# ORNL-Fusion/graph_framework

Measured on AMD Instinct MI355X. Metric: ray-steps/sec on xrays_bench cold-plasma; achieved HBM GB/s vs peak, higher is better.
Workload: dtype f64

## Files before the change

graph_framework_amd/build.py:

```python
import glob
import os
import subprocess

from . import _lib

HIPCC = os.environ.get("HIPCC", "/opt/rocm/bin/hipcc")
KERNEL_FLAGS = ["-O3", "-ffp-contract=off", "-fno-slp-vectorize", "--offload-arch=gfx950"]


def build_library(force=False):
    csrc = os.path.join(_lib.HERE, "csrc")
    sources = glob.glob(os.path.join(csrc, "*")) + glob.glob(os.path.join(_lib.HERE, "..", "include", "*.h"))
    newest = max(os.path.getmtime(s) for s in sources)
    programs = [os.path.join(_lib.HERE, name) for name in ("xrays_bench", "solver_check", "korc_push")]
    sources.append(os.path.join(_lib.HERE, "gf_workflow.hpp"))
    newest = max(os.path.getmtime(s) for s in sources)
    if (force or not os.path.exists(_lib.LIB_PATH) or os.path.getmtime(_lib.LIB_PATH) < newest
            or any(not os.path.exists(p) or os.path.getmtime(p) < newest for p in programs)):
        subprocess.check_call(["make", "-C", csrc, "-s", "HIPCC=" + HIPCC])
    return _lib.LIB_PATH


def compile_source(source, source_hash, force=False):
    os.makedirs(_lib.CACHE_DIR, exist_ok=True)
    stem = os.path.join(_lib.CACHE_DIR, "%016x" % source_hash)
    if force or not os.path.exists(stem + ".hsaco"):
        with open(stem + ".hip", "w") as f:
            f.write(source)
        subprocess.check_call([HIPCC, "--genco"] + KERNEL_FLAGS + ["-o", stem + ".hsaco", stem + ".hip"])
    return stem + ".hsaco"


def prebuild_kernel(gfir_path, force=False):
    from . import backend
    return [compile_source(source, source_hash, force) for source, source_hash in backend.generate_piece_sources(gfir_path)]


VARIANTS = [({"GFHIP_DIVISION": "fast"}, "solver_kernel_f64"), ({"GFHIP_DIVISION": "fast"}, "loss_kernel_kx_f64"),
            ({"GFHIP_ASM": "0"}, "solver_kernel_f64")]


def variant_sources():
    import json
    import sys
    texts = []
    for overrides, stem in VARIANTS:
        env = dict(os.environ)
        env.update(overrides)
        out = subprocess.run([sys.executable, "-c",
                              "import sys, json; sys.path.insert(0, %r)\n"
                              "from graph_framework_amd.backend import generate_piece_sources\n"
                              "print(json.dumps(generate_piece_sources(%r)))"
                              % (os.path.dirname(_lib.HERE), os.path.join(_lib.WORKLOAD_DIR, stem + ".gfir"))],
                             env=env, capture_output=True, text=True, check=True)
        texts += [tuple(piece) for piece in json.loads(out.stdout)]
    return texts


def prebuild_workloads(force=False):
    from concurrent.futures import ThreadPoolExecutor
    from . import backend
    paths = sorted(glob.glob(os.path.join(_lib.WORKLOAD_DIR, "*.gfir")))
# ... 15 lines not shown
```

graph_framework_amd/csrc/asm_body.hpp:

```cpp
#ifndef gfhip_asm_body_hpp
#define gfhip_asm_body_hpp

#include <algorithm>
#include <cstdint>
#include <cstdio>
#include <cstring>
#include <map>
#include <set>
#include <sstream>
#include <string>
#include <tuple>
#include <vector>

#include "gfir_item.hpp"
#include "options.hpp"
#include "schedule.hpp"
#include "tables.hpp"

namespace gfhip {

struct asm_body_text {
    bool ok = false;
    std::string why;
    std::string statement;
    uint32_t slots = 0;
    size_t vector = 0, scalar = 0, lds_reads = 0, lds_writes = 0, loads = 0, waits = 0;
};

class asm_body_writer {
    const item &it;
    const codegen_options &opt;
    const std::vector<pack> &packs;
    const std::vector<int> &parent;
    const std::vector<double> &factor;
    const std::vector<uint32_t> &table_pack, &table_column;
    const uint32_t block_size;
    const uint32_t slot_limit;
// ... 150 lines not shown
        used_at.assign(n, std::vector<int64_t> ());
        node_group.assign(n, -1);
        for (size_t i = 0; i < n; i++) {
            const gfir_instruction &c = it.code[i];
            alias[i] = static_cast<int64_t> (i);
            if (c.op == GFIR_GATHER1 || c.op == GFIR_GATHER2) {
                const table &t = it.tables[c.aux];
                const bool two = c.op == GFIR_GATHER2;
                const group_key key(c.a, two ? c.b : GFIR_NONE, t.rows, t.cols, c.imm[0], c.imm[1], two ? c.imm[2] : 0.0, two ? c.imm[3] : 0.0);
                auto found = group_of_key.find(key);
                if (found == group_of_key.end()) {
                    group g;
                    g.pack = table_pack[c.aux];
                    groups.push_back(g);
                    found = group_of_key.insert({key, static_cast<int> (groups.size()) - 1}).first;
                }
                node_group[i] = found->second;
                alias[i] = cell_value(found->second, c.aux);
            }
        }
        std::vector<bool> group_seen(groups.size(), false);
        for (size_t i = 0; i < n; i++) {
            const gfir_instruction &c = it.code[i];
            if (c.op == GFIR_CONST || c.op == GFIR_INPUT) continue;
            if (c.op == GFIR_GATHER1 || c.op == GFIR_GATHER2) {
                const size_t g = static_cast<size_t> (node_group[i]);
                if (!group_seen[g]) {
                    group_seen[g] = true;
                    if (it.code[c.a].op != GFIR_CONST) add_use(alias[c.a], i);
                    if (c.op == GFIR_GATHER2 && it.code[c.b].op != GFIR_CONST) add_use(alias[c.b], i);
                }
                continue;
            }
            const uint32_t operands[3] = {c.a, c.b, c.c};
            for (int k = 0; k < operand_count(c.op); k++) {
                if (it.code[operands[k]].op != GFIR_CONST) add_use(alias[operands[k]], i);
            }
            if (c.op == GFIR_DIV) add_use(static_cast<int64_t> (n + c.b), i);
        }
        for (auto &st : it.setters) {
            if (it.code[st.value].op != GFIR_CONST) add_use(alias[st.value], n);
        }
        for (auto o : it.outputs) {
            if (it.code[o].op != GFIR_CONST) add_use(alias[o], n);
        }
        for (size_t k = 2*n; k < values.size(); k++) {
            int64_t child = static_cast<int64_t> (k);
// ... 452 lines not shown
                vector_op("v_mad_u32_u24 " + low_name(cell) + ", " + low_name(index[0]) + ", " + std::to_string(t.cols) + ", " + low_name(index[1]));
            } else {
                vector_op("v_mul_u32_u24_e32 " + low_name(cell) + ", " + hex32(t.cols) + ", " + low_name(index[0]));
                vector_op("v_add_u32_e32 " + low_name(cell) + ", " + low_name(cell) + ", " + low_name(index[1]));
            }
            release_pair(index[1]);
        }
        const std::string defines = "def g" + std::to_string(node_group[i]) + " node " + std::to_string(i) + " stride " + std::to_string(pk.stride*8u) +
                                    " pack " + std::to_string(g.pack) + " lds " + std::to_string(pk.in_lds ? 1 : 0);
        if (!pk.in_lds) annotate(defines);
        vector_op("v_mul_u32_u24_e32 " + low_name(cell) + ", " + hex32(pk.stride*8u) + ", " + low_name(cell));
        if (pk.in_lds) {
            annotate(defines);
            vector_op("v_add_u32_e32 " + low_name(cell) + ", %[lds" + std::to_string(g.pack) + "], " + low_name(cell));
        }
        g.offset_pair = cell;
        owner[static_cast<size_t> (cell)] = -2;
    }

    void node(const size_t i) {
        const gfir_instruction &c = it.code[i];
        position = i;
        pinned.clear();
        look_ahead();
        std::vector<int64_t> read = used_at[i];
        switch (c.op) {
            case GFIR_CONST:
                return;
            case GFIR_INPUT:
                values[i].operand = "%[v" + std::to_string(c.a) + "]";
                values[i].defined = true;
                return;
            case GFIR_GATHER1:
            case GFIR_GATHER2:
                if (groups[static_cast<size_t> (node_group[i])].offset_pair == -1) find_cell(i);
                line("; alias r" + std::to_string(i) + " = " + value_name(alias[i]));
                break;
            case GFIR_ADD:
            case GFIR_SUB:
            case GFIR_MUL:
            case GFIR_FMA: {
                operands x = c.op == GFIR_FMA ? resolve({c.a, c.b, c.c}) : resolve({c.a, c.b}, {false, c.op == GFIR_SUB});
                retire(read);
                read.clear();
                const int p = need_pair();
                const char *name = c.op == GFIR_MUL ? "v_mul_f64 " : c.op == GFIR_FMA ? "v_fma_f64 " : "v_add_f64 ";
// ... 201 lines not shown
                if (k) s << ", ";
                s << "[park" << k << "] \"v\"(park" << k << ")";
            }
        }
        s << "\n                : ";
        for (uint32_t r = pool_lo; r < 256; r++) s << "\"v" << r << "\", ";
        for (int r = sgpr_lo; r < sgpr_lo + 2*sgpr_pairs; r++) s << "\"s" << r << "\", ";
        s << "\"memory\");\n";
        result.statement = s.str();
        result.ok = true;
        return result;
    }
};

inline item schedule_for_assembly(const item &in, const codegen_options &opt, const std::vector<std::string> &directories = {}) {
    if (in.code.size() > 20000 || !asm_body_writer::why_not(in, opt).empty()) return schedule_for_pressure(in);
    if (const char *forced = std::getenv("GFHIP_ASM_SEED")) {
        return reorder(in, list_schedule(in, static_cast<uint32_t> (std::atoi(forced))));
    }
    const std::vector<uint8_t> bytes = in.serialize();
    const uint64_t key = fnv1a(std::string(bytes.begin(), bytes.end()) + "|order|" + std::to_string(opt.asm_pool_lo) + "|" +
                               std::to_string(opt.asm_load_ahead) + "|" + std::to_string(opt.asm_reload_ahead) + "|" +
                               std::to_string(opt.asm_schedule_tries) + "|" + std::to_string(opt.asm_wide_loads) + "|" +
                               std::to_string(opt.lds_budget) + "|" + std::to_string(opt.compact_tables) + "|" + std::to_string(opt.block_size));
    char name[40];
    std::snprintf(name, sizeof(name), "/%016llx.order", static_cast<unsigned long long> (key));
    for (auto &directory : directories) {
        if (FILE *f = std::fopen((directory + name).c_str(), "r")) {
            unsigned int seed = 0;
            const bool read = std::fscanf(f, "%u", &seed) == 1;
            std::fclose(f);
            if (read) return reorder(in, list_schedule(in, seed));
        }
    }
    const table_layout layout = layout_tables(in, opt);
    item best;
    uint32_t best_seed = 0;
    size_t best_slots = ~static_cast<size_t> (0), best_traffic = 0;
    const uint32_t tries = in.code.size() <= 5000 ? opt.asm_schedule_tries
                         : std::max<uint32_t> (4u, static_cast<uint32_t> (opt.asm_schedule_tries*5000ull/in.code.size()));
    for (uint32_t seed = 0; seed < std::max(1u, tries); seed++) {
        item candidate = reorder(in, list_schedule(in, seed));
        asm_body_writer writer(candidate, opt, layout.packs, layout.parent, layout.factor, layout.table_pack, layout.table_column,
                               opt.block_size, 1u << 20);
        const asm_body_text text = writer.write();
        if (!text.ok) continue;
        const size_t traffic = text.lds_reads + text.lds_writes;
        if (std::getenv("GFHIP_ASM_REPORT")) {
            std::fprintf(stderr, "  order %u of %s: %u slots, %zu LDS reads, %zu LDS writes, %zu loads, %zu waits\n", seed, in.name.c_str(), text.slots,
                         text.lds_reads, text.lds_writes, text.loads, text.waits);
        }
        if (text.slots < best_slots || (text.slots == best_slots && traffic < best_traffic)) {
            best_slots = text.slots;
            best_traffic = traffic;
            best = std::move(candidate);
            best_seed = seed;
        }
    }
    if (best.code.empty()) return schedule_for_pressure(in);
    for (auto &directory : directories) {
        if (FILE *f = std::fopen((directory + name).c_str(), "w")) {
            std::fprintf(f, "%u\n", best_seed);
            std::fclose(f);
            break;
        }
    }
// ... 16 lines not shown
```

graph_framework_amd/csrc/codegen.hpp:

```cpp
#ifndef gfhip_codegen_hpp
#define gfhip_codegen_hpp

#include <algorithm>
#include <cmath>
#include <cstdint>
#include <cstdio>
#include <cstdlib>
#include <functional>
#include <map>
#include <set>
#include <sstream>
#include <string>
#include <tuple>
#include <vector>

#include "asm_body.hpp"
#include "gfir_item.hpp"
#include "options.hpp"
#include "parking.hpp"
#include "prelude.hpp"
#include "schedule.hpp"
#include "tables.hpp"

namespace gfhip {
// ... 129 lines not shown
            [&] (const std::string &group, const uint32_t t) -> std::string {
            const std::string value_name = "c" + group.substr(1) + "_" + std::to_string(t);
            if (coefficients.insert(value_name).second) {
                if (parent[t] >= 0) {
                    const std::string from = value_at(group, static_cast<uint32_t> (parent[t]));
                    s << ind << "const real " << value_name << " = " << literal(factor[t]) << "*" << from << ";\n";
                } else {
                    s << ind << "const real " << value_name << " = " << group << "[" << table_column[t] << "u];\n";
                }
            }
            return value_name;
        };
        std::map<uint32_t, std::pair<std::string, uint32_t>> deferred;
        auto define = [&] (const uint32_t v) {
            auto found = deferred.find(v);
            if (found == deferred.end()) return;
            const std::string value = value_at(found->second.first, found->second.second);
            s << ind << "const real r" << v << " = " << value << ";\n";
            deferred.erase(found);
        };
        for (size_t i = 0; i < it.code.size(); i++) {
            const gfir_instruction &c = it.code[i];
            reload(i);
            {
                const uint32_t operands[3] = {c.a, c.b, c.c};
                for (int k = 0; k < operand_count(c.op); k++) define(operands[k]);
            }
            switch (c.op) {
                case GFIR_CONST:
                    s << ind << "const real r" << i << " = " << value_literal(c.imm[0], c.imm[1]) << ";\n";
                    break;
                case GFIR_RANDOM:
                    s << ind << "const real r" << i << " = gf_from_base(static_cast<base> (gf_random(random_state)));\n";
                    break;
                case GFIR_INPUT:
                    s << ind << "const real r" << i << " = v" << c.a << ";\n";
                    break;
                case GFIR_ADD:
                    s << ind << "const real r" << i << " = " << N(c.a) << " + " << N(c.b) << ";\n";
                    break;
                case GFIR_SUB:
                    s << ind << "const real r" << i << " = " << N(c.a) << " - " << N(c.b) << ";\n";
                    break;
                case GFIR_MUL:
                    s << ind << "const real r" << i << " = ";
                    if (safe) s << "(" << N(c.a) << " == " << value_literal(0.0) << " || " << N(c.b) << " == " << value_literal(0.0) << ") ? " << value_literal(0.0) << " : ";
// ... 498 lines not shown
          << "        const real other = __shfl_down(" << lane << ", offset, 64);\n"
          << "        " << lane << " = other > " << lane << " ? other : " << lane << ";\n"
          << "    }\n"
          << "    __shared__ real " << scratch << "[" << out.block_size/64 << "];\n"
          << "    if ((threadIdx.x & 63u) == 0u) " << scratch << "[threadIdx.x >> 6] = " << lane << ";\n"
          << "    __syncthreads();\n"
          << "    if (threadIdx.x == 0u) {\n"
          << "        real block_max = " << scratch << "[0];\n"
          << "        for (unsigned int w = 1; w < (blockDim.x >> 6); w++) block_max = " << scratch << "[w] > block_max ? " << scratch << "[w] : block_max;\n"
          << "        const " << bits << " b = __builtin_bit_cast(" << bits << ", block_max);\n"
          << "        const " << bits << " top = static_cast<" << bits << "> (1) << " << (f64 ? 63 : 31) << ";\n"
          << "        atomicMax(" << target << ", static_cast<unsigned long long> (block_max != block_max ? static_cast<" << bits << "> (~static_cast<" << bits << "> (0))\n"
          << "                                                             : (b & top) ? static_cast<" << bits << "> (~b) : (b | top)));\n"
          << "    }\n";
    }
};

inline lowered lower(const item &original, const codegen_options &opt = codegen_options::from_environment(),
                     const piece_info &piece = piece_info()) {
    item scheduled;
    if (opt.schedule_for_pressure && !(opt.asm_body && piece.scheduled)) {
        scheduled = schedule_for_pressure(original);
    }
    const item &it = scheduled.code.empty() ? original : scheduled;
    lowered out;
    const size_t esize = it.element_size();

    out.input_written.assign(it.symbols.size(), false);
    for (auto &s : it.setters) {
        out.input_written[s.input] = true;
    }

    const table_layout layout = layout_tables(it, opt);
    const std::vector<int> &parent = layout.parent;
    const std::vector<double> &factor = layout.factor;
    const std::vector<uint32_t> &table_pack = layout.table_pack, &table_column = layout.table_column;
    out.table_parent = parent;
    out.table_factor = factor;
    out.packs = layout.packs;
    size_t lds_used = layout.lds_used;
    out.block_size = opt.block_size;

    const bool generic = it.is_complex() || it.safe_math() || it.has_random();
    codegen_options plain = opt;
    if (generic) plain.park_in_lds = false;
    asm_body_text assembly;
// ... 77 lines not shown
```

graph_framework_amd/csrc/gf_hip.cpp:

```cpp
#include <hip/hip_runtime.h>
#include <hip/hiprtc.h>

#include <dlfcn.h>
#include <sys/stat.h>

#include <cmath>
#include <complex>
#include <cstdio>
#include <cstdlib>
#include <cstring>
#include <fstream>
#include <limits>
#include <map>
#include <memory>
#include <optional>
#include <string>
#include <type_traits>
#include <vector>

#include "../../include/gf_hip.h"
#include "codegen.hpp"
#include "segments.hpp"

#include "converge_state.hpp"
#include "superacc.hpp"

namespace gfhip {
void launch_max_reduce(const void *in, const size_t n, const bool f64,
                       unsigned long long *result, const unsigned int num_cus, hipStream_t stream);
void launch_converge_decide(const bool f64, unsigned long long *reduced, void *state, hipStream_t stream);
void launch_converge_decide_batch(const bool f64, unsigned long long *reduced, void *state, const unsigned int count, hipStream_t stream);
void launch_max_modulus(const void *in, const size_t n, const bool f64, void *result, hipStream_t stream);
void launch_deposit(const double *x, const double *y, const double *z, const double *value, const size_t count,
                    const double *edges, const int nx, const int ny, const int nz, const double *scale,
                    void *state, unsigned long long *counters, const unsigned int num_cus, hipStream_t stream);
void launch_bins_normalise(void *state, const size_t cells, hipStream_t stream);
void launch_bins_round(const void *state, const size_t cells, const double divisor, double *bins, hipStream_t stream);
void launch_bins_merge(void *state, const void *other, const size_t words, hipStream_t stream);
}

namespace {

thread_local std::string creation_error;

// ... 234 lines not shown

static uint32_t plan_item(const gfhip::item &it, gfhip::lowered &whole, std::vector<built_piece> &pieces,
                          std::optional<built_piece> *redo = nullptr) {
    const gfhip::codegen_options opt = gfhip::codegen_options::from_environment();
    size_t count = 1;
    bool automatic = false;
    if (gfhip::can_split(it)) {
        if (opt.segments >= 1 && it.code.size() >= opt.segments_min_nodes && it.code.size() >= 2*opt.segments) {
            count = opt.segments;
        } else if (opt.segment_nodes && it.code.size() > opt.segment_nodes) {
            count = (it.code.size() + opt.segment_nodes - 1)/opt.segment_nodes;
            automatic = true;
        }
    }
    bool as_assembly = opt.asm_body && count < 2 && opt.segments == 0 && opt.schedule_for_pressure && gfhip::can_split(it) &&
                       it.code.size() >= opt.asm_min_nodes && opt.division == gfhip::division_mode::shared &&
                       gfhip::asm_body_writer::why_not(it, opt).empty();
    gfhip::item ordered;
    if (as_assembly) {
        std::vector<std::string> directories;
        if (const char *env = std::getenv("GFHIP_CACHE_DIR")) directories.push_back(env);
        directories.push_back(library_directory() + "/kernel_cache");
        ordered = gfhip::schedule_for_assembly(it, opt, directories);
        as_assembly = gfhip::assembly_fits(ordered, opt);
    }
    if (count < 2 && opt.segments != 1 && !as_assembly) {
        whole = gfhip::lower(it, opt);
        return 0;
    }
    if (!as_assembly) ordered = opt.schedule_for_pressure ? gfhip::schedule_for_pressure(it) : it;
    gfhip::segmentation plan = gfhip::split_item(ordered, gfhip::choose_cuts(ordered, count));
    if (plan.segments.size() == 1) plan.segments[0].piece.name = it.name;
    gfhip::codegen_options piece_options = opt;
    if (automatic) piece_options.division = gfhip::division_mode::ieee;
    const bool with_redo = !automatic && piece_options.division != gfhip::division_mode::ieee;
    std::vector<bool> after_division(ordered.code.size(), false);
    for (size_t i = 0; i < ordered.code.size(); i++) {
        const gfir_instruction &c = ordered.code[i];
        const uint32_t operands[3] = {c.a, c.b, c.c};
        bool dependent = c.op == GFIR_DIV;
        for (int k = 0; k < gfhip::operand_count(c.op) && !dependent; k++) dependent = after_division[operands[k]];
        after_division[i] = dependent;
    }
    for (size_t p = 0; p < plan.segments.size(); p++) {
        built_piece piece;
        gfhip::piece_info role;
        role.scheduled = opt.schedule_for_pressure;
        if (with_redo) {
            role.role = p + 1 == plan.segments.size() ? gfhip::piece_role::last : gfhip::piece_role::middle;
            for (auto slot : plan.segments[p].output_slot) role.output_handed_over.push_back(slot >= 0);
            for (auto record : plan.segments[p].symbol_record) role.symbol_after_division.push_back(record >= 0 && after_division[record]);
        }
        piece.low = gfhip::lower(plan.segments[p].piece, piece_options, role);
// ... 1228 lines not shown
```

graph_framework_amd/csrc/gfir_item.hpp:

```cpp
#ifndef gfir_item_hpp
#define gfir_item_hpp

#include <cctype>
#include <cstdint>
#include <cstring>
#include <string>
#include <vector>

#include "../../include/gfir.h"

namespace gfhip {

struct table {
    uint32_t rows, cols;
    std::vector<double> data;
};

struct item {
    uint32_t dtype = GFIR_F64;
    uint32_t flags = 0;
    std::string name;
    std::vector<std::string> symbols;
    std::vector<table> tables;
    std::vector<gfir_instruction> code;
    std::vector<uint32_t> outputs;
    std::vector<gfir_setter> setters;

    static size_t element_size(const uint32_t dtype) {
        return dtype == GFIR_F32 ? 4 : dtype == GFIR_C64 ? 16 : 8;
    }
    size_t element_size() const { return element_size(dtype); }
    bool is_complex() const { return dtype == GFIR_C32 || dtype == GFIR_C64; }
    bool base_is_f64() const { return dtype == GFIR_F64 || dtype == GFIR_C64; }
    bool safe_math() const { return flags & GFIR_SAFE_MATH; }
    bool has_random() const {
        for (auto &c : code) {
            if (c.op == GFIR_RANDOM) return true;
        }
        return false;
    }

    size_t indexed_length(const uint32_t i) const {
        size_t length = 0;
        for (auto &c : code) {
            if ((c.op == GFIR_INDEX1 || c.op == GFIR_INDEX2) && c.c == i) {
                const size_t needed = c.op == GFIR_INDEX1 ? c.aux : static_cast<size_t> (c.aux)*c.reserved;
                if (needed > length) length = needed;
            }
        }
// ... 187 lines not shown
```

graph_framework_amd/csrc/options.hpp:

```cpp
#ifndef gfhip_options_hpp
#define gfhip_options_hpp

#include <cstdint>
#include <cstdlib>
#include <string>

namespace gfhip {

enum class division_mode {
    shared,
    checked,
    ieee,
    fast
};

struct codegen_options {
    size_t lds_budget = 64*1024;
    uint32_t block_size = 256;
    uint32_t waves_per_simd = 0;
    division_mode division = division_mode::shared;
    bool pow_three_halves = true;
    bool window_sqrt = false;
    bool window_sqrt_f32 = true;
    int nontemporal = -1;
    bool compact_tables = true;
    bool park_in_lds = true;
    uint32_t park_min_range = 1500;
    uint32_t park_window = 100;
    uint32_t park_max_slots = 32;
    uint32_t park_prefetch = 50;
    uint32_t park_capacity = 0;
    bool schedule_for_pressure = true;
    int division_fixup = -1;
    uint32_t converge_batch = 3;
    uint32_t segment_nodes = 6000;
    uint32_t segments = 0;
    uint32_t segments_min_nodes = 2000;
    bool asm_body = true;
    uint32_t asm_waves = 2;
    bool asm_wide_loads = true;
    uint32_t asm_schedule_tries = 64;
    uint32_t asm_min_nodes = 1000;
    uint32_t asm_pool_lo = 40;
    uint32_t asm_load_ahead = 96;
    uint32_t asm_reload_ahead = 24;
    size_t handover_bytes = 128u << 20;

    static codegen_options from_environment() {
        codegen_options o;
        if (const char *e = std::getenv("GFHIP_DIVISION")) {
            const std::string mode(e);
            o.division = mode == "ieee" ? division_mode::ieee : mode == "checked" ? division_mode::checked
                       : mode == "fast" ? division_mode::fast : division_mode::shared;
        }
        if (const char *e = std::getenv("GFHIP_PARK")) {
            const std::string mode(e);
            o.park_in_lds = mode != "0";
            if (mode == "heavy") o.park_min_range = 300;
        }
        if (const char *e = std::getenv("GFHIP_SCHEDULE")) o.schedule_for_pressure = std::string(e) != "source";
        if (const char *e = std::getenv("GFHIP_DIV_FIXUP")) o.division_fixup = std::string(e) != "0" ? 1 : 0;
        if (const char *e = std::getenv("GFHIP_NONTEMPORAL")) o.nontemporal = std::atoi(e);
        if (const char *e = std::getenv("GFHIP_COMPACT_TABLES")) o.compact_tables = std::string(e) != "0";
        if (const char *e = std::getenv("GFHIP_POW")) o.pow_three_halves = std::string(e) != "libm";
        if (const char *e = std::getenv("GFHIP_PARK_CAPACITY")) o.park_capacity = static_cast<uint32_t> (std::atoi(e));
        if (const char *e = std::getenv("GFHIP_PARK_PREFETCH")) o.park_prefetch = static_cast<uint32_t> (std::atoi(e));
        if (const char *e = std::getenv("GFHIP_ASM")) o.asm_body = std::string(e) != "0";
        if (const char *e = std::getenv("GFHIP_ASM_WAVES")) o.asm_waves = static_cast<uint32_t> (std::atoi(e)) == 2 ? 2 : 1;
        if (const char *e = std::getenv("GFHIP_ASM_WIDE_LOADS")) o.asm_wide_loads = std::string(e) != "0";
        if (const char *e = std::getenv("GFHIP_ASM_TRIES")) o.asm_schedule_tries = static_cast<uint32_t> (std::atoi(e));
        if (const char *e = std::getenv("GFHIP_ASM_MIN_NODES")) o.asm_min_nodes = static_cast<uint32_t> (std::atoi(e));
        if (const char *e = std::getenv("GFHIP_ASM_POOL_LO")) o.asm_pool_lo = static_cast<uint32_t> (std::atoi(e));
        if (const char *e = std::getenv("GFHIP_ASM_LOAD_AHEAD")) o.asm_load_ahead = static_cast<uint32_t> (std::atoi(e));
        if (const char *e = std::getenv("GFHIP_ASM_RELOAD_AHEAD")) o.asm_reload_ahead = static_cast<uint32_t> (std::atoi(e));
        if (const char *e = std::getenv("GFHIP_WINDOW_SQRT")) o.window_sqrt = std::string(e) == "1";
        if (const char *e = std::getenv("GFHIP_WINDOW_SQRT_F32")) o.window_sqrt_f32 = std::string(e) == "1";
        if (const char *e = std::getenv("GFHIP_WAVES_PER_SIMD")) o.waves_per_simd = static_cast<uint32_t> (std::atoi(e));
        if (const char *e = std::getenv("GFHIP_LDS_BUDGET")) o.lds_budget = static_cast<size_t> (std::atol(e));
        if (const char *e = std::getenv("GFHIP_CONVERGE_BATCH")) o.converge_batch = static_cast<uint32_t> (std::atol(e) > 0 ? std::atol(e) : 1);
        if (o.converge_batch > 8) o.converge_batch = 8;
        if (const char *e = std::getenv("GFHIP_SEGMENT_NODES")) o.segment_nodes = static_cast<uint32_t> (std::atol(e));
        if (const char *e = std::getenv("GFHIP_SEGMENTS")) o.segments = static_cast<uint32_t> (std::atol(e));
        if (const char *e = std::getenv("GFHIP_SEGMENTS_MIN_NODES")) o.segments_min_nodes = static_cast<uint32_t> (std::atol(e));
        if (const char *e = std::getenv("GFHIP_HANDOVER_BYTES")) o.handover_bytes = static_cast<size_t> (std::atoll(e));
        return o;
    }
};

inline uint64_t fnv1a(const std::string &s) {
    uint64_t h = 1469598103934665603ull;
    for (unsigned char c : s) {
        h ^= c;
        h *= 1099511628211ull;
    }
    return h;
}

inline const char *compile_flags() {
    return "-O3 -ffp-contract=off -fno-slp-vectorize --offload-arch=gfx950";
}

}

#endif
```

graph_framework_amd/csrc/schedule.hpp:

```cpp
#ifndef gfhip_schedule_hpp
#define gfhip_schedule_hpp

#include <set>
#include <vector>

#include "gfir_item.hpp"

namespace gfhip {

inline int operand_count(const uint32_t op) {
    switch (op) {
        case GFIR_CONST: case GFIR_INPUT: return 0;
        case GFIR_FMA: return 3;
        case GFIR_SQRT: case GFIR_POWI: case GFIR_SIN: case GFIR_COS: case GFIR_EXP: case GFIR_LOG: case GFIR_ERFI:
        case GFIR_GATHER1: case GFIR_INDEX1: case GFIR_RANDOM: return 1;
        default: return 2;
    }
}

inline item reorder(const item &in, const std::vector<uint32_t> &order) {
    const size_t n = in.code.size();
    std::vector<uint32_t> new_index(n, GFIR_NONE);
    for (size_t p = 0; p < order.size(); p++) new_index[order[p]] = static_cast<uint32_t> (p);
    item out = in;
    for (size_t p = 0; p < order.size(); p++) {
        gfir_instruction c = in.code[order[p]];
        const int count = operand_count(c.op);
        if (count > 0) c.a = new_index[c.a];
        if (count > 1) c.b = new_index[c.b];
        if (count > 2) c.c = new_index[c.c];
        out.code[p] = c;
    }
    for (auto &s : out.setters) s.value = new_index[s.value];
    for (auto &o : out.outputs) o = new_index[o];
    return out;
}

inline item schedule_for_pressure(const item &in) {
    const size_t n = in.code.size();
    if (n > 20000) return in;
    std::vector<std::vector<uint32_t>> users(n);
    std::vector<uint32_t> pending(n, 0), consumers_left(n, 0);
    std::vector<bool> is_root(n, false);
    for (auto &s : in.setters) is_root[s.value] = true;
    for (auto o : in.outputs) is_root[o] = true;
    for (size_t i = 0; i < n; i++) {
        const gfir_instruction &c = in.code[i];
        const uint32_t operands[3] = {c.a, c.b, c.c};
        std::set<uint32_t> distinct;
        for (int k = 0; k < operand_count(c.op); k++) distinct.insert(operands[k]);
        pending[i] = static_cast<uint32_t> (distinct.size());
        for (auto o : distinct) {
            users[o].push_back(static_cast<uint32_t> (i));
            consumers_left[o]++;
        }
    }

    std::vector<uint32_t> distinct_operands(3*n, GFIR_NONE);
    std::vector<uint8_t> distinct_count(n, 0);
    for (size_t i = 0; i < n; i++) {
        const gfir_instruction &c = in.code[i];
        const uint32_t operands[3] = {c.a, c.b, c.c};
        for (int k = 0; k < operand_count(c.op); k++) {
            bool seen = false;
            for (int j = 0; j < distinct_count[i]; j++) seen = seen || distinct_operands[3*i + j] == operands[k];
            if (!seen) distinct_operands[3*i + distinct_count[i]++] = operands[k];
        }
    }

    std::set<uint32_t> ready;
    std::vector<uint32_t> stamp(n, 0);
    for (size_t i = 0; i < n; i++) {
        if (pending[i] == 0) ready.insert(static_cast<uint32_t> (i));
    }
    std::vector<uint32_t> order;
    order.reserve(n);
    while (!ready.empty()) {
        uint32_t best = *ready.begin();
        int best_score = 1 << 30;
        for (const uint32_t v : ready) {
            int freed = 0;
            for (int k = 0; k < distinct_count[v]; k++) {
                const uint32_t o = distinct_operands[3*static_cast<size_t> (v) + k];
                if (in.code[o].op != GFIR_CONST && consumers_left[o] == 1 && !is_root[o]) freed++;
            }
            const int grows = (in.code[v].op == GFIR_CONST) ? 0 : 1;
            const int score = grows - freed;
            if (score < best_score || (score == best_score && stamp[v] > stamp[best])) {
                best_score = score;
                best = v;
            }
        }
        ready.erase(best);
        order.push_back(best);
        for (int k = 0; k < distinct_count[best]; k++) consumers_left[distinct_operands[3*static_cast<size_t> (best) + k]]--;
        for (auto u : users[best]) {
            if (--pending[u] == 0) {
                ready.insert(u);
                stamp[u] = static_cast<uint32_t> (order.size());
            }
        }
    }

    return reorder(in, order);
}

inline std::vector<uint32_t> list_schedule(const item &in, const uint32_t seed) {
    const size_t n = in.code.size();
    uint64_t state = 0x9E3779B97F4A7C15ull*(seed + 1u);
    auto next = [&state] () {
        uint64_t z = (state += 0x9E3779B97F4A7C15ull);
        z = (z ^ (z >> 30))*0xBF58476D1CE4E5B9ull;
        z = (z ^ (z >> 27))*0x94D049BB133111EBull;
        return z ^ (z >> 31);
    };
    std::vector<std::vector<uint32_t>> users(n);
    std::vector<uint32_t> pending(n, 0), consumers_left(n, 0);
    std::vector<bool> is_root(n, false);
    for (auto &s : in.setters) is_root[s.value] = true;
    for (auto o : in.outputs) is_root[o] = true;
    std::vector<uint32_t> distinct_operands(3*n, GFIR_NONE);
    std::vector<uint8_t> distinct_count(n, 0);
    for (size_t i = 0; i < n; i++) {
        const gfir_instruction &c = in.code[i];
        const uint32_t operands[3] = {c.a, c.b, c.c};
        for (int k = 0; k < operand_count(c.op); k++) {
            bool seen = false;
            for (int j = 0; j < distinct_count[i]; j++) seen = seen || distinct_operands[3*i + j] == operands[k];
            if (!seen) distinct_operands[3*i + distinct_count[i]++] = operands[k];
        }
        pending[i] = distinct_count[i];
        for (int k = 0; k < distinct_count[i]; k++) {
            users[distinct_operands[3*i + k]].push_back(static_cast<uint32_t> (i));
            consumers_left[distinct_operands[3*i + k]]++;
        }
    }
    std::set<uint32_t> ready;
    std::vector<uint32_t> stamp(n, 0), order, best;
    for (size_t i = 0; i < n; i++) {
        if (pending[i] == 0) ready.insert(static_cast<uint32_t> (i));
    }
    order.reserve(n);
    while (!ready.empty()) {
        best.clear();
        int best_score = 1 << 30;
        uint32_t best_stamp = 0;
        for (const uint32_t v : ready) {
            int freed = 0;
            for (int k = 0; k < distinct_count[v]; k++) {
                const uint32_t o = distinct_operands[3*static_cast<size_t> (v) + k];
                if (in.code[o].op != GFIR_CONST && consumers_left[o] == 1 && !is_root[o]) freed++;
            }
            const int score = (in.code[v].op == GFIR_CONST ? 0 : 1) - freed;
            if (score < best_score || (score == best_score && stamp[v] > best_stamp)) {
                best_score = score;
                best_stamp = stamp[v];
                best.clear();
            }
            if (score == best_score && stamp[v] == best_stamp) best.push_back(v);
        }
        const uint32_t pick = best[static_cast<size_t> (next()%best.size())];
        ready.erase(pick);
        order.push_back(pick);
        for (int k = 0; k < distinct_count[pick]; k++) consumers_left[distinct_operands[3*static_cast<size_t> (pick) + k]]--;
        for (auto u : users[pick]) {
            if (--pending[u] == 0) {
                ready.insert(u);
                stamp[u] = static_cast<uint32_t> (order.size());
            }
        }
    }
    return order;
}

}

#endif
```

graph_framework_amd/csrc/segments.hpp:

```cpp
#ifndef gfhip_segments_hpp
#define gfhip_segments_hpp

#include <algorithm>
#include <cstdint>
#include <map>
#include <set>
#include <string>
#include <vector>

#include "gfir_item.hpp"
#include "options.hpp"
#include "schedule.hpp"

namespace gfhip {

struct segment {
    item piece;
    std::vector<int> symbol_state;
    std::vector<int> symbol_slot;
    std::vector<int> symbol_record;
    std::vector<int> output_slot;
    std::vector<int> output_original;
};

struct segmentation {
    std::vector<segment> segments;
    uint32_t slots = 0;
    std::vector<size_t> cuts;
    std::vector<size_t> crossing;
};

inline bool can_split(const item &it) {
    if (it.is_complex() || it.safe_math() || it.has_random()) return false;
    for (auto &c : it.code) {
        if (c.op == GFIR_INDEX1 || c.op == GFIR_INDEX2) return false;
    }
    return !it.code.empty();
}

inline std::vector<size_t> choose_cuts(const item &it, const size_t count, const double window = 0.45) {
    const size_t n = it.code.size();
    std::vector<size_t> last_use(n, 0);
    for (size_t i = 0; i < n; i++) {
        const gfir_instruction &c = it.code[i];
        const uint32_t operands[3] = {c.a, c.b, c.c};
        for (int k = 0; k < operand_count(c.op); k++) last_use[operands[k]] = i;
    }
    for (auto &s : it.setters) last_use[s.value] = n;
    for (auto o : it.outputs) last_use[o] = n;
    std::vector<int> delta(n + 2, 0);
    for (size_t v = 0; v < n; v++) {
        const uint32_t op = it.code[v].op;
        if (op == GFIR_CONST || op == GFIR_INPUT || last_use[v] <= v) continue;
        delta[v + 1]++;
        delta[std::min(last_use[v], n) + 1]--;
    }
    std::vector<int> alive(n + 1, 0);
    int running = 0;
    for (size_t p = 0; p <= n; p++) {
        running += delta[p];
        alive[p] = running;
    }
    std::vector<size_t> cuts;
    const double length = static_cast<double> (n)/static_cast<double> (count);
    for (size_t k = 1; k < count; k++) {
        const double centre = length*static_cast<double> (k);
        size_t low = static_cast<size_t> (std::max(1.0, centre - window*length));
        size_t high = static_cast<size_t> (std::min(static_cast<double> (n - 1), centre + window*length));
        if (!cuts.empty() && low <= cuts.back()) low = cuts.back() + 1;
// ... 9 lines not shown

inline segmentation split_item(const item &it, const std::vector<size_t> &cuts) {
    const size_t n = it.code.size();
    segmentation result;
    result.cuts = cuts;
    std::vector<size_t> bounds = {0};
    for (auto c : cuts) bounds.push_back(c);
    bounds.push_back(n);
    const size_t count = bounds.size() - 1;
    auto segment_of = [&] (const size_t record) -> size_t {
        return static_cast<size_t> (std::upper_bound(bounds.begin(), bounds.end(), record) - bounds.begin()) - 1;
    };

    std::vector<size_t> last_segment(n, 0);
    std::vector<bool> used_later(n, false);
    auto use = [&] (const uint32_t value, const size_t by) {
        const uint32_t op = it.code[value].op;
        if (op == GFIR_CONST || op == GFIR_INPUT) return;
        if (by > segment_of(value)) {
            used_later[value] = true;
            last_segment[value] = std::max(last_segment[value], by);
        }
    };
    for (size_t i = 0; i < n; i++) {
        const gfir_instruction &c = it.code[i];
        const uint32_t operands[3] = {c.a, c.b, c.c};
        for (int k = 0; k < operand_count(c.op); k++) use(operands[k], segment_of(i));
    }
    for (auto &s : it.setters) use(s.value, count - 1);
    for (auto o : it.outputs) use(o, count - 1);

    std::vector<int> slot_of(n, -1);
    std::vector<size_t> slot_free_after;
    for (size_t v = 0; v < n; v++) {
        if (!used_later[v]) continue;
        const size_t defined = segment_of(v);
        int slot = -1;
        for (size_t k = 0; k < slot_free_after.size(); k++) {
            if (slot_free_after[k] < defined) { slot = static_cast<int> (k); break; }
        }
        if (slot < 0) {
            slot = static_cast<int> (slot_free_after.size());
            slot_free_after.push_back(0);
        }
        slot_free_after[slot] = last_segment[v];
        slot_of[v] = slot;
    }
    result.slots = static_cast<uint32_t> (slot_free_after.size());
    for (auto c : cuts) {
        size_t crossing = 0;
// ... 34 lines not shown
            slot_symbol[slot] = index;
            return index;
        };
        if (k == count - 1) {
            for (auto &s : it.setters) (void)symbol_for_state(s.input);
        }
        std::function<uint32_t(uint32_t)> resolve = [&] (const uint32_t value) -> uint32_t {
            auto found = local.find(value);
            if (found != local.end()) return found->second;
            const gfir_instruction &c = it.code[value];
            gfir_instruction fresh = c;
            if (c.op == GFIR_INPUT) {
                fresh.a = symbol_for_state(c.a);
            } else if (c.op != GFIR_CONST) {
                fresh = gfir_instruction();
                fresh.op = GFIR_INPUT;
                fresh.a = symbol_for_slot(slot_of[value], value);
                fresh.b = fresh.c = GFIR_NONE;
            }
            piece.code.push_back(fresh);
            local[value] = static_cast<uint32_t> (piece.code.size() - 1);
            return local[value];
        };
        for (size_t i = bounds[k]; i < bounds[k + 1]; i++) {
            gfir_instruction c = it.code[i];
            if (c.op == GFIR_INPUT) {
                c.a = symbol_for_state(c.a);
            } else {
                const int operands = operand_count(c.op);
                if (operands > 0) c.a = resolve(c.a);
                if (operands > 1) c.b = resolve(c.b);
                if (operands > 2) c.c = resolve(c.c);
                if (c.op == GFIR_GATHER1 || c.op == GFIR_GATHER2) {
                    auto found = table_local.find(c.aux);
                    if (found == table_local.end()) {
                        piece.tables.push_back(it.tables[c.aux]);
                        found = table_local.insert({c.aux, static_cast<uint32_t> (piece.tables.size() - 1)}).first;
                    }
                    c.aux = found->second;
                }
            }
            piece.code.push_back(c);
            local[static_cast<uint32_t> (i)] = static_cast<uint32_t> (piece.code.size() - 1);
        }
        for (size_t i = bounds[k]; i < bounds[k + 1]; i++) {
            if (used_later[i]) {
                piece.outputs.push_back(local[static_cast<uint32_t> (i)]);
                seg.output_slot.push_back(slot_of[i]);
                seg.output_original.push_back(-1);
            }
        }
        if (k == count - 1) {
            for (auto &s : it.setters) {
                gfir_setter moved;
                moved.value = resolve(s.value);
                moved.input = symbol_for_state(s.input);
                piece.setters.push_back(moved);
            }
            for (size_t o = 0; o < it.outputs.size(); o++) {
                piece.outputs.push_back(resolve(it.outputs[o]));
                seg.output_slot.push_back(-1);
                seg.output_original.push_back(static_cast<int> (o));
            }
        }
        result.segments.push_back(std::move(seg));
    }
    return result;
}

}

#endif
```

Before: 5.732 billion.

## Add value-numbering merge of duplicate arithmetic records and powi prefix reuse

Adds a global value-numbering pass that detects duplicate add/sub/mul/fma/div/powi records and aliases them to the first computation. It also rewrites integer powers to reuse an existing lower-power prefix. The scheduler, segment splitter, asm writer and C++ codegen are taught to carry the alias map, and the pass is on by default with an env switch. It aims to cut redundant vector arithmetic in the generated solver kernels, at the risk of longer live ranges and more register pressure.

```diff
diff --git a/graph_framework_amd/build.py b/graph_framework_amd/build.py
--- a/graph_framework_amd/build.py
+++ b/graph_framework_amd/build.py
@@ -37,7 +37,7 @@
 
 
 VARIANTS = [({"GFHIP_DIVISION": "fast"}, "solver_kernel_f64"), ({"GFHIP_DIVISION": "fast"}, "loss_kernel_kx_f64"),
-            ({"GFHIP_ASM": "0"}, "solver_kernel_f64")]
+            ({"GFHIP_ASM": "0"}, "solver_kernel_f64"), ({"GFHIP_MERGE": "0"}, "solver_kernel_f64")]
 
 
 def variant_sources():
diff --git a/graph_framework_amd/csrc/asm_body.hpp b/graph_framework_amd/csrc/asm_body.hpp
--- a/graph_framework_amd/csrc/asm_body.hpp
+++ b/graph_framework_amd/csrc/asm_body.hpp
@@ -13,6 +13,7 @@
 #include <vector>
 
 #include "gfir_item.hpp"
+#include "merge.hpp"
 #include "options.hpp"
 #include "schedule.hpp"
 #include "tables.hpp"
@@ -209,7 +210,7 @@
         std::vector<bool> group_seen(groups.size(), false);
         for (size_t i = 0; i < n; i++) {
             const gfir_instruction &c = it.code[i];
-            if (c.op == GFIR_CONST || c.op == GFIR_INPUT) continue;
+            if (c.op == GFIR_CONST || c.op == GFIR_INPUT || it.is_merged(i)) continue;
             if (c.op == GFIR_GATHER1 || c.op == GFIR_GATHER2) {
                 const size_t g = static_cast<size_t> (node_group[i]);
                 if (!group_seen[g]) {
@@ -708,6 +709,10 @@
         const gfir_instruction &c = it.code[i];
         position = i;
         pinned.clear();
+        if (it.is_merged(i)) {
+            line("; alias r" + std::to_string(i) + " = r" + std::to_string(it.merged_into[i]));
+            return;
+        }
         look_ahead();
         std::vector<int64_t> read = used_at[i];
         switch (c.op) {
@@ -955,7 +960,8 @@
     const uint64_t key = fnv1a(std::string(bytes.begin(), bytes.end()) + "|order|" + std::to_string(opt.asm_pool_lo) + "|" +
                                std::to_string(opt.asm_load_ahead) + "|" + std::to_string(opt.asm_reload_ahead) + "|" +
                                std::to_string(opt.asm_schedule_tries) + "|" + std::to_string(opt.asm_wide_loads) + "|" +
-                               std::to_string(opt.lds_budget) + "|" + std::to_string(opt.compact_tables) + "|" + std::to_string(opt.block_size));
+                               std::to_string(opt.lds_budget) + "|" + std::to_string(opt.compact_tables) + "|" + std::to_string(opt.block_size) +
+                               (opt.merge ? "|merged" : ""));
     char name[40];
     std::snprintf(name, sizeof(name), "/%016llx.order", static_cast<unsigned long long> (key));
     for (auto &directory : directories) {
@@ -974,7 +980,8 @@
                          : std::max<uint32_t> (4u, static_cast<uint32_t> (opt.asm_schedule_tries*5000ull/in.code.size()));
     for (uint32_t seed = 0; seed < std::max(1u, tries); seed++) {
         item candidate = reorder(in, list_schedule(in, seed));
-        asm_body_writer writer(candidate, opt, layout.packs, layout.parent, layout.factor, layout.table_pack, layout.table_column,
+        const item merged = opt.merge ? merge_records(candidate) : item();
+        asm_body_writer writer(opt.merge ? merged : candidate, opt, layout.packs, layout.parent, layout.factor, layout.table_pack, layout.table_column,
                                opt.block_size, 1u << 20);
         const asm_body_text text = writer.write();
         if (!text.ok) continue;
diff --git a/graph_framework_amd/csrc/codegen.hpp b/graph_framework_amd/csrc/codegen.hpp
--- a/graph_framework_amd/csrc/codegen.hpp
+++ b/graph_framework_amd/csrc/codegen.hpp
@@ -175,6 +175,10 @@
         for (size_t i = 0; i < it.code.size(); i++) {
             const gfir_instruction &c = it.code[i];
             reload(i);
+            if (it.is_merged(i)) {
+                s << ind << "const real r" << i << " = " << N(it.merged_into[i]) << ";\n";
+                continue;
+            }
             {
                 const uint32_t operands[3] = {c.a, c.b, c.c};
                 for (int k = 0; k < operand_count(c.op); k++) define(operands[k]);
@@ -719,6 +723,11 @@
     if (opt.schedule_for_pressure && !(opt.asm_body && piece.scheduled)) {
         scheduled = schedule_for_pressure(original);
     }
+    if (opt.merge && (piece.role == piece_role::none || piece.role == piece_role::redo) && original.merged_into.empty()) {
+        merge_report merges;
+        scheduled = merge_records(scheduled.code.empty() ? original : scheduled, &merges);
+        if (std::getenv("GFHIP_ASM_REPORT")) merges.print(stderr, original.name);
+    }
     const item &it = scheduled.code.empty() ? original : scheduled;
     lowered out;
     const size_t esize = it.element_size();
diff --git a/graph_framework_amd/csrc/gf_hip.cpp b/graph_framework_amd/csrc/gf_hip.cpp
--- a/graph_framework_amd/csrc/gf_hip.cpp
+++ b/graph_framework_amd/csrc/gf_hip.cpp
@@ -20,6 +20,7 @@
 
 #include "../../include/gf_hip.h"
 #include "codegen.hpp"
+#include "merge.hpp"
 #include "segments.hpp"
 
 #include "converge_state.hpp"
@@ -300,13 +301,18 @@
         if (const char *env = std::getenv("GFHIP_CACHE_DIR")) directories.push_back(env);
         directories.push_back(library_directory() + "/kernel_cache");
         ordered = gfhip::schedule_for_assembly(it, opt, directories);
-        as_assembly = gfhip::assembly_fits(ordered, opt);
+        as_assembly = gfhip::assembly_fits(opt.merge ? gfhip::merge_records(ordered) : ordered, opt);
     }
     if (count < 2 && opt.segments != 1 && !as_assembly) {
         whole = gfhip::lower(it, opt);
         return 0;
     }
     if (!as_assembly) ordered = opt.schedule_for_pressure ? gfhip::schedule_for_pressure(it) : it;
+    if (opt.merge) {
+        gfhip::merge_report merges;
+        ordered = gfhip::merge_records(ordered, &merges);
+        if (std::getenv("GFHIP_ASM_REPORT")) merges.print(stderr, it.name);
+    }
     gfhip::segmentation plan = gfhip::split_item(ordered, gfhip::choose_cuts(ordered, count));
     if (plan.segments.size() == 1) plan.segments[0].piece.name = it.name;
     gfhip::codegen_options piece_options = opt;
diff --git a/graph_framework_amd/csrc/gfir_item.hpp b/graph_framework_amd/csrc/gfir_item.hpp
--- a/graph_framework_amd/csrc/gfir_item.hpp
+++ b/graph_framework_amd/csrc/gfir_item.hpp
@@ -25,6 +25,9 @@
     std::vector<gfir_instruction> code;
     std::vector<uint32_t> outputs;
     std::vector<gfir_setter> setters;
+    std::vector<uint32_t> merged_into;
+
+    bool is_merged(const size_t record) const { return !merged_into.empty() && merged_into[record] != GFIR_NONE; }
 
     static size_t element_size(const uint32_t dtype) {
         return dtype == GFIR_F32 ? 4 : dtype == GFIR_C64 ? 16 : 8;
diff --git a/graph_framework_amd/csrc/merge.hpp b/graph_framework_amd/csrc/merge.hpp
--- /dev/null
+++ b/graph_framework_amd/csrc/merge.hpp
@@ -0,0 +1,166 @@
+#ifndef gfhip_merge_hpp
+#define gfhip_merge_hpp
+
+#include <cstdint>
+#include <cstdio>
+#include <cstring>
+#include <string>
+#include <unordered_map>
+#include <utility>
+#include <vector>
+
+#include "gfir_item.hpp"
+#include "schedule.hpp"
+
+namespace gfhip {
+
+struct merge_report {
+    size_t add = 0, sub = 0, mul = 0, fma = 0, div = 0, powi = 0;
+    size_t prefixes = 0;
+    size_t instructions = 0;
+    std::vector<std::pair<uint32_t, uint32_t>> merged;
+    std::vector<std::pair<uint32_t, uint32_t>> prefixed;
+
+    size_t records() const { return add + sub + mul + fma + div + powi; }
+    void print(FILE *out, const std::string &name) const {
+        std::fprintf(out, "merge of %s: %zu records merged (add %zu, sub %zu, mul %zu, fma %zu, div %zu, powi %zu), %zu powi prefixes, "
+                          "%zu vector instructions\n", name.c_str(), records(), add, sub, mul, fma, div, powi, prefixes, instructions);
+        for (auto &m : merged) std::fprintf(out, "  merged r%u into r%u\n", m.first, m.second);
+        for (auto &p : prefixed) std::fprintf(out, "  powi r%u from its prefix r%u\n", p.first, p.second);
+    }
+};
+
+inline bool can_merge(const item &it) {
+    if (it.is_complex() || it.safe_math() || it.has_random()) return false;
+    for (auto &c : it.code) {
+        if (c.op == GFIR_INDEX1 || c.op == GFIR_INDEX2) return false;
+    }
+    return true;
+}
+
+inline item merge_records(const item &in, merge_report *report = nullptr) {
+    if (!can_merge(in)) return in;
+    const size_t n = in.code.size();
+
+    struct key {
+        uint32_t op, a, b, c, aux;
+        uint64_t imm[4];
+        bool operator==(const key &o) const {
+            return op == o.op && a == o.a && b == o.b && c == o.c && aux == o.aux && std::memcmp(imm, o.imm, sizeof(imm)) == 0;
+        }
+    };
+    struct key_hash {
+        size_t operator()(const key &k) const {
+            uint64_t h = 1469598103934665603ull;
+            auto mix = [&h] (const uint64_t v) { h = (h ^ v)*1099511628211ull; h ^= h >> 29; };
+            mix(k.op); mix(k.a); mix(k.b); mix(k.c); mix(k.aux);
+            for (const uint64_t v : k.imm) mix(v);
+            return static_cast<size_t> (h);
+        }
+    };
+    std::unordered_map<key, uint32_t, key_hash> numbers;
+    numbers.reserve(2*n);
+    std::vector<uint32_t> holder;
+    auto number_of = [&] (const key &k) -> uint32_t {
+        auto found = numbers.find(k);
+        if (found != numbers.end()) return found->second;
+        holder.push_back(GFIR_NONE);
+        numbers.insert({k, static_cast<uint32_t> (holder.size() - 1)});
+        return static_cast<uint32_t> (holder.size() - 1);
+    };
+    auto plain = [] (const uint32_t op, const uint32_t a, const uint32_t b = GFIR_NONE, const uint32_t c = GFIR_NONE, const uint32_t aux = 0) {
+        key k;
+        k.op = op; k.a = a; k.b = b; k.c = c; k.aux = aux;
+        std::memset(k.imm, 0, sizeof(k.imm));
+        return k;
+    };
+
+    item out = in;
+    std::vector<uint32_t> value(n, GFIR_NONE);
+    std::vector<uint32_t> stands(n);
+    std::vector<uint32_t> merged_into(n, GFIR_NONE);
+    merge_report counts;
+    for (size_t i = 0; i < n; i++) {
+        gfir_instruction &c = out.code[i];
+        stands[i] = static_cast<uint32_t> (i);
+        const int operands = operand_count(c.op);
+        uint32_t va = GFIR_NONE, vb = GFIR_NONE, vc = GFIR_NONE;
+        if (operands > 0) { va = value[c.a]; c.a = stands[c.a]; }
+        if (operands > 1) { vb = value[c.b]; c.b = stands[c.b]; }
+        if (operands > 2) { vc = value[c.c]; c.c = stands[c.c]; }
+        bool mergeable = false;
+        uint32_t id, prefix = GFIR_NONE;
+        switch (c.op) {
+            case GFIR_CONST: {
+                key k = plain(c.op, GFIR_NONE);
+                std::memcpy(k.imm, c.imm, 2*sizeof(uint64_t));
+                id = number_of(k);
+                break;
+            }
+            case GFIR_INPUT:
+                id = number_of(plain(c.op, c.a));
+                break;
+            case GFIR_GATHER1: case GFIR_GATHER2: {
+                key k = plain(c.op, va, vb, GFIR_NONE, c.aux);
+                std::memcpy(k.imm, c.imm, sizeof(k.imm));
+                id = number_of(k);
+                break;
+            }
+            case GFIR_POWI:
+                if (c.aux < 2) {
+                    id = number_of(plain(c.op, va, GFIR_NONE, GFIR_NONE, c.aux));
+                    break;
+                }
+                id = number_of(plain(GFIR_MUL, va, va));
+                for (uint32_t p = 3; p <= c.aux; p++) {
+                    prefix = id;
+                    id = number_of(plain(GFIR_MUL, prefix, va));
+                }
+                mergeable = true;
+                break;
+            case GFIR_ADD: case GFIR_SUB: case GFIR_MUL: case GFIR_DIV: case GFIR_FMA:
+                mergeable = true;
+                id = number_of(plain(c.op, va, vb, vc));
+                break;
+            default:
+                id = number_of(plain(c.op, va, vb, vc));
+        }
+        value[i] = id;
+        if (holder[id] == GFIR_NONE) {
+            holder[id] = static_cast<uint32_t> (i);
+            if (c.op == GFIR_POWI && prefix != GFIR_NONE && holder[prefix] != GFIR_NONE) {
+                counts.prefixes++;
+                counts.instructions += c.aux - 2;
+                counts.prefixed.push_back({static_cast<uint32_t> (i), holder[prefix]});
+                c.op = GFIR_MUL;
+                c.b = c.a;
+                c.a = holder[prefix];
+                c.aux = 0;
+            }
+            continue;
+        }
+        if (!mergeable) continue;
+        const uint32_t first = holder[id];
+        switch (c.op) {
+            case GFIR_ADD: counts.add++; counts.instructions += 1; break;
+            case GFIR_SUB: counts.sub++; counts.instructions += 1; break;
+            case GFIR_MUL: counts.mul++; counts.instructions += 1; break;
+            case GFIR_FMA: counts.fma++; counts.instructions += 1; break;
+            case GFIR_DIV: counts.div++; counts.instructions += 3; break;
+            default: counts.powi++; counts.instructions += c.aux - 1;
+        }
+        counts.merged.push_back({static_cast<uint32_t> (i), first});
+        c = out.code[first];
+        stands[i] = first;
+        merged_into[i] = first;
+    }
+    for (auto &s : out.setters) s.value = stands[s.value];
+    for (auto &o : out.outputs) o = stands[o];
+    if (counts.records()) out.merged_into = merged_into;
+    if (report) *report = counts;
+    return out;
+}
+
+}
+
+#endif
diff --git a/graph_framework_amd/csrc/options.hpp b/graph_framework_amd/csrc/options.hpp
--- a/graph_framework_amd/csrc/options.hpp
+++ b/graph_framework_amd/csrc/options.hpp
@@ -44,6 +44,7 @@
     uint32_t asm_pool_lo = 40;
     uint32_t asm_load_ahead = 96;
     uint32_t asm_reload_ahead = 24;
+    bool merge = true;
     size_t handover_bytes = 128u << 20;
 
     static codegen_options from_environment() {
@@ -82,6 +83,7 @@
         if (const char *e = std::getenv("GFHIP_SEGMENT_NODES")) o.segment_nodes = static_cast<uint32_t> (std::atol(e));
         if (const char *e = std::getenv("GFHIP_SEGMENTS")) o.segments = static_cast<uint32_t> (std::atol(e));
         if (const char *e = std::getenv("GFHIP_SEGMENTS_MIN_NODES")) o.segments_min_nodes = static_cast<uint32_t> (std::atol(e));
+        if (const char *e = std::getenv("GFHIP_MERGE")) o.merge = std::string(e) != "0";
         if (const char *e = std::getenv("GFHIP_HANDOVER_BYTES")) o.handover_bytes = static_cast<size_t> (std::atoll(e));
         return o;
     }
diff --git a/graph_framework_amd/csrc/schedule.hpp b/graph_framework_amd/csrc/schedule.hpp
--- a/graph_framework_amd/csrc/schedule.hpp
+++ b/graph_framework_amd/csrc/schedule.hpp
@@ -33,6 +33,9 @@
     }
     for (auto &s : out.setters) s.value = new_index[s.value];
     for (auto &o : out.outputs) o = new_index[o];
+    for (size_t p = 0; p < order.size() && !in.merged_into.empty(); p++) {
+        out.merged_into[p] = in.is_merged(order[p]) ? new_index[in.merged_into[order[p]]] : GFIR_NONE;
+    }
     return out;
 }
 
@@ -44,8 +47,14 @@
     std::vector<bool> is_root(n, false);
     for (auto &s : in.setters) is_root[s.value] = true;
     for (auto o : in.outputs) is_root[o] = true;
+    std::vector<std::vector<uint32_t>> names(in.merged_into.empty() ? 0 : n);
     for (size_t i = 0; i < n; i++) {
         const gfir_instruction &c = in.code[i];
+        if (in.is_merged(i)) {
+            names[in.merged_into[i]].push_back(static_cast<uint32_t> (i));
+            pending[i] = 1;
+            continue;
+        }
         const uint32_t operands[3] = {c.a, c.b, c.c};
         std::set<uint32_t> distinct;
         for (int k = 0; k < operand_count(c.op); k++) distinct.insert(operands[k]);
@@ -61,7 +70,7 @@
     for (size_t i = 0; i < n; i++) {
         const gfir_instruction &c = in.code[i];
         const uint32_t operands[3] = {c.a, c.b, c.c};
-        for (int k = 0; k < operand_count(c.op); k++) {
+        for (int k = 0; k < operand_count(c.op) && !in.is_merged(i); k++) {
             bool seen = false;
             for (int j = 0; j < distinct_count[i]; j++) seen = seen || distinct_operands[3*i + j] == operands[k];
             if (!seen) distinct_operands[3*i + distinct_count[i]++] = operands[k];
@@ -93,6 +102,7 @@
         }
         ready.erase(best);
         order.push_back(best);
+        if (!names.empty()) order.insert(order.end(), names[best].begin(), names[best].end());
         for (int k = 0; k < distinct_count[best]; k++) consumers_left[distinct_operands[3*static_cast<size_t> (best) + k]]--;
         for (auto u : users[best]) {
             if (--pending[u] == 0) {
@@ -121,8 +131,14 @@
     for (auto o : in.outputs) is_root[o] = true;
     std::vector<uint32_t> distinct_operands(3*n, GFIR_NONE);
     std::vector<uint8_t> distinct_count(n, 0);
+    std::vector<std::vector<uint32_t>> names(in.merged_into.empty() ? 0 : n);
     for (size_t i = 0; i < n; i++) {
         const gfir_instruction &c = in.code[i];
+        if (in.is_merged(i)) {
+            names[in.merged_into[i]].push_back(static_cast<uint32_t> (i));
+            pending[i] = 1;
+            continue;
+        }
         const uint32_t operands[3] = {c.a, c.b, c.c};
         for (int k = 0; k < operand_count(c.op); k++) {
             bool seen = false;
@@ -162,6 +178,7 @@
         const uint32_t pick = best[static_cast<size_t> (next()%best.size())];
         ready.erase(pick);
         order.push_back(pick);
+        if (!names.empty()) order.insert(order.end(), names[pick].begin(), names[pick].end());
         for (int k = 0; k < distinct_count[pick]; k++) consumers_left[distinct_operands[3*static_cast<size_t> (pick) + k]]--;
         for (auto u : users[pick]) {
             if (--pending[u] == 0) {
diff --git a/graph_framework_amd/csrc/segments.hpp b/graph_framework_amd/csrc/segments.hpp
--- a/graph_framework_amd/csrc/segments.hpp
+++ b/graph_framework_amd/csrc/segments.hpp
@@ -3,9 +3,11 @@
 
 #include <algorithm>
 #include <cstdint>
+#include <functional>
 #include <map>
 #include <set>
 #include <string>
+#include <utility>
 #include <vector>
 
 #include "gfir_item.hpp"
@@ -44,7 +46,7 @@
     for (size_t i = 0; i < n; i++) {
         const gfir_instruction &c = it.code[i];
         const uint32_t operands[3] = {c.a, c.b, c.c};
-        for (int k = 0; k < operand_count(c.op); k++) last_use[operands[k]] = i;
+        for (int k = 0; k < operand_count(c.op) && !it.is_merged(i); k++) last_use[operands[k]] = i;
     }
     for (auto &s : it.setters) last_use[s.value] = n;
     for (auto o : it.outputs) last_use[o] = n;
@@ -100,10 +102,13 @@
             last_segment[value] = std::max(last_segment[value], by);
         }
     };
+    auto name_of_representative = [&] (const size_t i) {
+        return it.is_merged(i) && segment_of(it.merged_into[i]) == segment_of(i);
+    };
     for (size_t i = 0; i < n; i++) {
         const gfir_instruction &c = it.code[i];
         const uint32_t operands[3] = {c.a, c.b, c.c};
-        for (int k = 0; k < operand_count(c.op); k++) use(operands[k], segment_of(i));
+        for (int k = 0; k < operand_count(c.op) && !it.is_merged(i); k++) use(operands[k], segment_of(i));
     }
     for (auto &s : it.setters) use(s.value, count - 1);
     for (auto o : it.outputs) use(o, count - 1);
@@ -184,9 +189,14 @@
             local[value] = static_cast<uint32_t> (piece.code.size() - 1);
             return local[value];
         };
+        std::vector<std::pair<uint32_t, uint32_t>> names;
         for (size_t i = bounds[k]; i < bounds[k + 1]; i++) {
             gfir_instruction c = it.code[i];
-            if (c.op == GFIR_INPUT) {
+            if (it.is_merged(i) && !name_of_representative(i)) {
+                c = gfir_instruction();
+                c.op = GFIR_CONST;
+                c.a = c.b = c.c = GFIR_NONE;
+            } else if (c.op == GFIR_INPUT) {
                 c.a = symbol_for_state(c.a);
             } else {
                 const int operands = operand_count(c.op);
@@ -204,6 +214,7 @@
             }
             piece.code.push_back(c);
             local[static_cast<uint32_t> (i)] = static_cast<uint32_t> (piece.code.size() - 1);
+            if (name_of_representative(i)) names.push_back({local[static_cast<uint32_t> (i)], local[it.merged_into[i]]});
         }
         for (size_t i = bounds[k]; i < bounds[k + 1]; i++) {
             if (used_later[i]) {
@@ -225,6 +236,10 @@
                 seg.output_original.push_back(static_cast<int> (o));
             }
         }
+        if (!names.empty()) {
+            piece.merged_into.assign(piece.code.size(), GFIR_NONE);
+            for (auto &name : names) piece.merged_into[name.first] = name.second;
+        }
         result.segments.push_back(std::move(seg));
     }
     return result;
```

After: 5.794 billion, median of 6. 1.01x the previous value.
